# athas/raytracers

Measured on AMD Instinct MI355X. Metric: Mray/s (primary+secondary) on rgbbox & irreg 1000x1000, higher is better.
Workload: dtype f32

## Files before the change

### raytracers_amd/csrc/api.cpp

```cpp
#include <hip/hip_runtime.h>

#include <algorithm>
#include <chrono>
#include <cmath>
#include <cstdio>
#include <cstdlib>
#include <cstring>
#include <memory>
#include <string>
#include <vector>

#include "../../include/rt_mi355x.h"
#include "rt_device.hpp"
#include "rt_host.hpp"
#include "rt_internal.hpp"

namespace rti {
int fail(rt_context *ctx, const std::string &msg) {
  if (ctx) ctx->err = msg;
  return 1;
}
int hip_fail(rt_context *ctx, hipError_t e, const char *what) {
  return fail(ctx, std::string(what) + ": " + hipGetErrorString(e));
}
// ... 402 lines not shown
  p->dark = (ctx->dark_stop != 0 && p->cost == nullptr && (!instrumented || ctx->dark_stop > 0)) ? 1 : 0;
}

void set_leaf_box(const rt_context *ctx, const rt_prepared *ps, const Plan &pl, const float *cams_dev, bool instrumented, rtk::KParams *p) {
  p->leaf_box = 0;
  if (ctx->leaf_box == 0 || !ps->leaf.ok || pl.variant != RT_VARIANT_POOLED || (instrumented && ctx->leaf_box <= 0)) return;
  if (pl.lds_nodes != p->n_nodes || pl.lds_sph != p->n_sph) return;
  if (cams_dev == nullptr ? !rt::leaf_box_camera_ok(ps->leaf, &p->cam.ox) : (cams_dev != ctx->cams_dev || ctx->cams_host == nullptr)) return;
  for (int f = 0; cams_dev != nullptr && f < p->nframes; ++f)
    if (!rt::leaf_box_camera_ok(ps->leaf, ctx->cams_host + 12 * f)) return;
  rtk::PooledKey k{};
  if (!rtk::choose_pooled(*p, instrumented, pl.waves, 0, &k) || !rtk::pooled_leaf_box(k)) return;
  p->leaf_box = 1;
}

std::string pooled_launch_name(const rtk::KParams &p, int waves, int rays = 0) {
  rtk::PooledKey k{};
  return rtk::choose_pooled(p, false, waves, rays, &k) ? rtk::pooled_name(k) : "none";
}
const char *pooled_launch_nodes(const rtk::KParams &p, int waves) {
  rtk::PooledKey k{};
  return rtk::choose_pooled(p, false, waves, 0, &k) && rtk::pooled_presort(k) ? "sign-ordered" : "planes";
}

void frame_params(const rt_prepared *ps, int64_t h, int64_t w, int rows_per_tile, int part, int nparts, int max_depth, const float *cam12, rtk::KParams *p) {
  scene_params(ps, p);
  std::memcpy(&p->cam, cam12 ? static_cast<const void *>(cam12) : static_cast<const void *>(&ps->cam), sizeof(p->cam));
  p->w = static_cast<int>(w); p->h = static_cast<int>(h);
  p->rows_local = static_cast<int>(rt::part_rows(h, rows_per_tile, part, nparts));
  p->rows_per_tile = rows_per_tile; p->part = part; p->nparts = nparts;
  p->rpt_log2 = (rows_per_tile & (rows_per_tile - 1)) == 0 ? __builtin_ctz(rows_per_tile) : -1;
  p->tiles_x = (p->w + 7) / 8;
  p->tiles_y = (p->rows_local + 7) / 8;
  p->max_depth = max_depth;
  p->nframes = 1;
}

bool twenty_waves(const rt_context *ctx, const Plan &pl) { return pl.waves * (pl.grid_full / std::max(1, ctx->num_cu)) == 20; }

int pooled_shape_params(rt_context *ctx, const rt_prepared *ps, const Plan &pl, rtk::KParams *p) {
  p->static_first = ctx->static_first;
  p->lds_nodes = pl.lds_nodes; p->lds_sph = pl.lds_sph;
  p->smax = pl.smax; p->lmax = pl.lmax;
  p->thr_shade = ctx->thr_shade; p->thr_leaf = ctx->thr_leaf;
  p->capb = pl.capb; p->capl = pl.capl; p->ray_planes = pl.ray_planes;
  if (pl.spill_stride > 0) {
    if (int rc = ensure_spill(ctx, pl.spill_stride)) return rc;
    p->spill = ctx->spill_dev;
    p->spill_stride = pl.spill_stride;
  }
  p->prio_depth = ctx->prio_depth;
  p->box2 = ctx->box2;
  p->look_max = ctx->look_max > 0 ? ctx->look_max : (twenty_waves(ctx, pl) ? 16 : (p->nframes > 1 || p->nchunks > 16384) ? 32 : 64);
  p->tl_log2 = ps->tl_depth;
  return 0;
}

// ... 218 lines not shown
int rti::pooled_rays_params(rt_context *ctx, const rt_prepared *ps, const Plan &pl, rtk::KParams *pp) {
  rtk::KParams &p = *pp;
  if (ps->n >= (int64_t(1) << 22)) return fail(ctx, "pooled kernel: at most 2^22 spheres (work items and hit keys carry the leaf index in 22 bits)");
  const int64_t nblocks = (static_cast<int64_t>(p.nrays) + 63) / 64;
  p.nframes = 1;
  p.queue = ctx->queue_dev;
  p.w = 64; p.h = 1;
  p.rows_local = 1; p.rows_per_tile = 1; p.part = 0; p.nparts = 1; p.rpt_log2 = 0;
  p.tiles_x = static_cast<int>(nblocks); p.tiles_y = 1;
  p.nchunks = static_cast<int>(nblocks);
  p.tpt_log2 = 0;
  set_counters(&p, ctx->xcd_queues != 0 ? 2 : 0, pl.grid);
  return pooled_shape_params(ctx, ps, pl, &p);
}

int rti::launch_pooled_rays(rt_context *ctx, const rtk::KParams &p, const Plan &pl, int rays) {
  RT_HIP(ctx, rtk::launch_pooled(p, false, pl.grid, pl.waves, ctx->stream, rays));
  char buf[256];
  std::snprintf(buf, sizeof buf, "family=pooled tickets=rays instantiation=%s frames=1 tiles=%d grid=%d waves=%d counters=%d%s deep_class=0 deep_split=0 recording=0%s",
                pooled_launch_name(p, pl.waves, rays).c_str(), p.nchunks, pl.grid, pl.waves, p.nshards, p.interleave ? "(turns)" : "",
                p.ray_tlo_dev != nullptr ? " intervals=per-ray" : "");
  ctx->last_launch = buf;
  return 0;
}

int rti::enqueue_render(rt_context *ctx, const rt_prepared *ps, int64_t h, int64_t w, int32_t max_depth, int32_t rows_per_tile,
                        int32_t part, int32_t nparts, int32_t *out_dev, bool stats, const float *cam12, int32_t nframes,
                        int64_t frame_stride, const float *cams_dev, bool inplace) {
  if (!ctx || !ps) return fail(ctx, "null context or prepared scene");
  RT_LOCK(ctx);
  RT_LOCK_PS(ps);
// ... 72 lines not shown
    ctx->last_launch = "family=persistent";
    return 0;
  }
  if (ps->n >= (int64_t(1) << 22)) return fail(ctx, "pooled kernel: at most 2^22 spheres (work items and hit keys carry the leaf index in 22 bits)");
  if (p.rpt_log2 < 0) return fail(ctx, "pooled kernel: rows_per_tile must be a power of two");
  if (int rc = get_uv(ctx, w, h, &p.u_tab, &p.v_tab)) return rc;
  tick("uv tables");
  TileOrder *to = nullptr;
  if (ctx->adaptive_order && !p.cams)
    if (int rc = find_view(ctx, ps, p, pl, &to)) return rc;
  Tickets t;
  if (int rc = choose_tickets(ctx, ps, to, xq, tick, p, pl, &t)) return rc;
  set_cull(ctx, ps, pl, cams_dev, &p);
  set_dark(ctx, false, &p);
  set_leaf_box(ctx, ps, pl, cams_dev, false, &p);
  tick("before launch");
  RT_HIP(ctx, rtk::launch_pooled(p, false, pl.grid, pl.waves, ctx->stream));
  tick("launch_pooled");
  char buf[320];
  std::snprintf(buf, sizeof buf, "family=pooled tickets=%s%s instantiation=%s frames=%d tiles=%d grid=%d waves=%d counters=%d%s deep_class=%d deep_split=%d recording=%d nodes=%s,dark=%d,leaf_box=%d",
                p.px_hdr ? "pixel-list" : t.first_order ? "tiles-bit-reversed" : (p.order ? "tiles-ordered" : "tiles-raster"), t.borrowed ? "(borrowed)" : "",
                pooled_launch_name(p, pl.waves).c_str(), p.nframes, p.nchunks, pl.grid, pl.waves, p.nshards, p.interleave ? "(turns)" : "", p.px_hdr ? 0 : p.deep_class,
                p.px_hdr ? 0 : p.deep_split, p.cost ? (p.cost_px ? 2 : 1) : 0, pooled_launch_nodes(p, pl.waves), p.dark, p.leaf_box);
  ctx->last_launch = buf;
  if (to && p.cost) {
    to->sort_pending = true;
    to->sort_px = p.cost_px != nullptr;
    to->rec_out_skip = p.out_skip;
    if (ctx->eager_sort && (stream_was_idle || ctx->sync_policy))
      if (int rc = sort_view(ctx, ps, to, p, pl)) return rc;
    tick("record: eager sorts");
  }
  return 0;
}
using rti::enqueue_render;

extern "C" void rt_context_destroy(rt_context *ctx);

// ... 221 lines not shown
    ctx->px_solo_div = std::max(1, std::min(4096, v));
  } else if (k == "eager_sort") {
    drain_streams(ctx);
    ctx->eager_sort = v != 0;
  } else if (k == "borrow") {
    ctx->borrow = std::max(0, std::min(4, v));
  } else if (k == "stack_cap") {
    if (v != 0 && v != rtk::kSpillCapbTest) return fail(ctx, "stack_cap must be 0 or 192");
    ctx->stack_cap = v;
  } else if (k == "wide_waves") {
    ctx->wide_waves = std::max(0, std::min(2, v));
  } else if (k == "cull") {
    ctx->cull = std::max(-1, std::min(1, v));
  } else if (k == "dark_stop") {
    ctx->dark_stop = std::max(-1, std::min(1, v));
  } else if (k == "leaf_box") {
    ctx->leaf_box = std::max(-1, std::min(1, v));
  } else if (k == "sync_policy") {
    ctx->sync_policy = v != 0;
  } else {
    return fail(ctx, "unknown option: " + k);
  }
  return 0;
}

extern "C" int rt_context_device_info(const rt_context *ctx, int *device, int *num_cu, int *lds_bytes, char *name,
                                      int name_len) {
  RT_LOCK(const_cast<rt_context *>(ctx));
  if (!ctx) return 1;
  if (device) *device = ctx->device;
// ... 608 lines not shown
        p.deep_split = dp.deep_split;
        p.deep_cap_log2 = dp.cap_log2;
        if (dp.sparse && ctx->grid_div == 0) pl.grid = pl.grid_full;
        if (px_list_launch(ctx, p, pl, &o)) {
          p.px_list = o.px_list;
          p.px_hdr = reinterpret_cast<const int *>(o.px_list + o.px_elems);
          p.px_hold = ctx->px_hold;
          p.px_prio = ctx->px_prio;
          p.solo = (ctx->trace_solo && o.px_solo && ctx->solo && ps->tl_depth == rtk::kTreeletDepth) ? 1 : 0;
          if (ctx->grid_div == 0 && pl.grid != pl.grid_full && counters_follow(&p, xq, pl.grid_full)) pl.grid = pl.grid_full;
        }
      }
    nw = pl.grid * pl.waves;
    set_cull(ctx, ps, pl, nullptr, &p);
    set_dark(ctx, true, &p);
    set_leaf_box(ctx, ps, pl, nullptr, true, &p);
    e = rtk::launch_pooled(p, true, pl.grid, pl.waves, ctx->stream);
    if (e == hipSuccess) e = hipStreamSynchronize(ctx->stream);
    if (e == hipSuccess) e = hipMemcpy(records, trace, sizeof(unsigned long long) * rtk::kTraceWords * static_cast<size_t>(nw), hipMemcpyDeviceToHost);
  }
  (void)hipFree(tmp);
  (void)hipFree(trace);
  if (rc) return rc;
  if (e != hipSuccess) return hip_fail(ctx, e, "rt_render_trace");
  *num_waves = nw;
  return 0;
}

extern "C" int rt_render_timed(rt_context *ctx, const rt_prepared *ps, int64_t h, int64_t w, int32_t max_depth,
                               int32_t rows_per_tile, int32_t part, int32_t nparts, int32_t *out_dev, int32_t warmup,
// ... 58 lines not shown
```

### raytracers_amd/csrc/render_kernels.hip

```cpp
#include <hip/hip_runtime.h>

#include <mutex>
#include <type_traits>
#include <utility>

#include "lane_core.h"
#include "rt_device.hpp"
#include "treelet.h"

#ifdef RT_ISA_MARKS
#define RT_MARK(name) asm volatile("; RT_MARK " name)
#else
#define RT_MARK(name)
#endif

namespace rtk {

__device__ __forceinline__ int global_row(const KParams &p, int lrow) {
  const int k = lrow / p.rows_per_tile;
  return (k * p.nparts + p.part) * p.rows_per_tile + (lrow - k * p.rows_per_tile);
}

__device__ __forceinline__ size_t out_index(const KParams &p, int lrow, int col) {
  return (size_t)lrow * p.w + col + (size_t)(lrow / p.rows_per_tile) * (size_t)p.out_skip;
// ... 269 lines not shown
}

__device__ __forceinline__ float pull(int lane_byte, float v) {
  return __int_as_float(__builtin_amdgcn_ds_bpermute(lane_byte, __float_as_int(v)));
}

typedef const __attribute__((address_space(4))) KParams *KParamsArg;
typedef float v4f __attribute__((ext_vector_type(4)));
__device__ __forceinline__ float4 lds_load16(unsigned a) {
  const v4f v = *reinterpret_cast<const __attribute__((address_space(3))) v4f *>(a);
  return make_float4(v.x, v.y, v.z, v.w);
}
typedef float v2f __attribute__((ext_vector_type(2)));
typedef const __attribute__((address_space(3))) char *lds_cp;
__device__ __forceinline__ lds_cp lds_ptr(unsigned a) { return reinterpret_cast<lds_cp>(a); }
__device__ __forceinline__ v2f lds_load8(lds_cp a) { return *reinterpret_cast<const __attribute__((address_space(3))) v2f *>(a); }
__device__ __forceinline__ float lds_load4f(lds_cp a) { return *reinterpret_cast<const __attribute__((address_space(3))) float *>(a); }
#define RT_PS_NEAR(cell, t, entry) ((cell) + (t) + (entry))
#define RT_PS_FAR(cell, t, entry, dist) ((cell) - (t) + ((entry) + (int)(dist)))
__device__ __forceinline__ unsigned lds_load4(unsigned a) { return *reinterpret_cast<const __attribute__((address_space(3))) unsigned *>(a); }

constexpr bool kSoloCull = false;
template <bool CULL, bool TRACE = false>
__device__ __attribute__((noinline)) void solo_trace(KParamsArg pp_v, unsigned smem_lds, unsigned wbase_lds, float ox, float oy, float oz,
                                                     float dx, float dy, float dz, float lr, float lg, float lb, int pix, int depth,
                                                     int ptile) {
  const unsigned long long pp_bits = (unsigned long long)pp_v;
  KParamsArg pp = (KParamsArg)(((unsigned long long)(unsigned)uni((int)(pp_bits >> 32)) << 32) | (unsigned)uni((int)pp_bits));
  smem_lds = (unsigned)uni((int)smem_lds); wbase_lds = (unsigned)uni((int)wbase_lds);
  pix = uni(pix); depth = uni(depth); ptile = uni(ptile);
// ... 143 lines not shown
      return;
    }
  }
}

__device__ __forceinline__ int launch_dark() {
  return *reinterpret_cast<const volatile __attribute__((address_space(4))) int *>(&((KParamsArg)__builtin_amdgcn_kernarg_segment_ptr())->dark);
}

__device__ __forceinline__ unsigned long long launch_leaf_off() {
  KParamsArg kp = (KParamsArg)__builtin_amdgcn_kernarg_segment_ptr();
  asm volatile("" : "+s"(kp));
  return (unsigned long long)(unsigned)kp->leaf_box - 1ull;
}

template <int THREADS, bool ALL_LDS, bool STATS, bool SOLO, int TAIL = 0, bool ORD = false, bool CULL = false, int SPILL = 0, int RAYS = 0>
__global__ __launch_bounds__(THREADS, THREADS == 256 ? 5 : (THREADS / 64 + 3) / 4) void pooled_kernel(KParams p) {
  constexpr bool COLD = TAIL == 1, DONATE = TAIL == 2;
  constexpr bool ANY = RAYS == kRaysAny;
  static_assert(!RAYS || (!STATS && !SOLO && TAIL == 0 && !ORD && !CULL), "RAYS: the plain instantiations only");
  static_assert(!ORD || TAIL != 1, "ORD: no COLD variant");
  static_assert(!CULL || !ALL_LDS, "CULL: instantiated for the general scene path only");
  constexpr bool PRESORT = pooled_presort(ALL_LDS, SOLO, TAIL, ORD, RAYS);
  constexpr bool LEAFBOX = pooled_leaf_box(THREADS, ALL_LDS, STATS, SOLO, CULL, RAYS);
  extern __shared__ float4 smem[];
  const int lane = threadIdx.x & 63;
  const int wave = threadIdx.x >> 6;
  const int plane = p.lds_nodes;
  const int sph_base = 4 * plane;
  const int per_wave_dw = pooled_wave_dw(p.ray_planes, p.capb, p.capl);
  unsigned *const wbase = reinterpret_cast<unsigned *>(smem + sph_base + p.lds_sph) + wave * per_wave_dw;
  unsigned long long *const wkey = reinterpret_cast<unsigned long long *>(wbase);
  int *const wcnt = reinterpret_cast<int *>(wbase + 128);
  unsigned *const wdump = wbase + 192;
  float4 *const wray = reinterpret_cast<float4 *>(wbase + kPooledWaveFixedDw);
  unsigned *const wbox = wbase + kPooledWaveFixedDw + 256 * p.ray_planes;
  unsigned *const wleaf = wbox + p.capb;
  const __amdgpu_buffer_rsrc_t rs_nodes = make_rsrc(p.nodes64, (unsigned)p.n_nodes * 64u);
  const __amdgpu_buffer_rsrc_t rs_sph = make_rsrc(p.sph, (unsigned)p.n_sph * 16u);
  const __amdgpu_buffer_rsrc_t rs_col = make_rsrc(p.col, (unsigned)p.n_sph * 16u);

  if constexpr (PRESORT) {
    auto ref_of = [](float w) { const int c = f2i(w) >> 8; return (unsigned)(c < 0 ? c : c * kPsNodeBytes) << kPsItemShift; };
    for (int i = threadIdx.x; i < plane; i += THREADS) {
      const float4 ll = p.nodes64[4 * i], lh = p.nodes64[4 * i + 1], rl = p.nodes64[4 * i + 2], rh = p.nodes64[4 * i + 3];
      presort_pack(reinterpret_cast<unsigned *>(smem) + (kPsNodeBytes / 4) * i, &ll.x, &lh.x, &rl.x, &rh.x, ref_of(ll.w), ref_of(lh.w));
    }
  } else {
    for (int i = threadIdx.x; i < 4 * plane; i += THREADS) smem[(i & 3) * plane + (i >> 2)] = p.nodes64[i];
  }
  for (int i = threadIdx.x; i < p.lds_sph; i += THREADS) smem[sph_base + i] = p.sph[i];
  for (int i = lane; i < per_wave_dw; i += 64) wbase[i] = 0u;
  unsigned *const wg_words = reinterpret_cast<unsigned *>(smem + sph_base + p.lds_sph) + 193;
  if (DONATE && threadIdx.x == 0) wg_words[1] = THREADS / 64;
  __syncthreads();
  wkey[lane] = kKeyInit;

  Ray r = {};
  float lr = 1.0f, lg = 1.0f, lb = 1.0f;
  int depth = 0;
  int pix = -1;
  unsigned long long n_rays = 0, n_box = 0, n_sph = 0;
  int nbox = 0, nleaf = 0;
  static_assert(!SPILL || (THREADS == 256 && !ALL_LDS && !SOLO && TAIL == 0 && !ORD), "SPILL: the plain and CULL kernels of the four-wave workgroups");
  unsigned *const wspill = wbase + 193;
  auto spill_region = [&]() { return p.spill + (size_t)(blockIdx.x * (THREADS / 64) + wave) * (size_t)p.spill_stride; };
  unsigned q_next = 0, q_end = 0;
  int q_tile = 0;
// ... 140 lines not shown
          bool root = false;
          if (STATS) tr_ops[2]++;
          const unsigned long long tr_s0 = STATS ? clock64() : 0ull;
          if constexpr (ANY) {
            if (done) {
              p.occluded[pix] = wkey[lane] == kKeyAnyHit ? 1 : 0;
              pix = -1;
            }
          } else if (done) {
            if (STATS) tr_maxdepth = depth > tr_maxdepth ? depth : tr_maxdepth;
            const unsigned long long key = wkey[lane];
            const float best = __uint_as_float((unsigned)(key >> 32));
            const bool hit = key != kKeyInit;
            const int bestj = (int)((unsigned)key >> 1);
            const int wj = hit ? bestj : 0;
            float4 c = buf_load16(rs_col, wj * 16), s;
            if (ALL_LDS) {
              s = smem[sph_base + wj];
            } else {
              s = smem[sph_base + (wj < p.lds_sph ? wj : 0)];
              if (wj >= p.lds_sph) s = buf_load16(rs_sph, wj * 16);
            }
            if (!hit) {
              s = make_float4(0.f, 0.f, 0.f, 1.f);
              c = make_float4(0.f, 0.f, 0.f, 0.f);
            }
            bool have = hit;
            float t = best;
            if (hit && !rehit_is_best(best, ((unsigned)key & 1u) != 0u)) have = rehit_full(r, best, s.x, s.y, s.z, s.w, &t);
            int32_t pixel;
            if constexpr (!SPILL) pixel = 0;
            bool more;
            if constexpr (RAYS)
// ... 91 lines not shown
                exhausted = true;
                if (STATS) tr_exh = wall_clock64();
                break;
              }
              q_next = sp.q_next;
              q_end = sp.q_end;
              q_enter = true;
            }
            if (__builtin_expect(q_enter || (q_next & 63u) == 0u, 0)) {
              q_enter = false;
              unsigned t = q_next >> 6;
              if (p.nframes > 1) {
                unsigned f;
                if (p.order != nullptr) {
                  const int *cb = p.order + p.nchunks;
                  unsigned c = 0;
                  while (c + 1 < (unsigned)kOrderClasses && t >= (unsigned)p.nframes * (unsigned)cb[c + 1]) ++c;
                  const unsigned base = (unsigned)cb[c], size = (unsigned)cb[c + 1] - base;
                  const unsigned within = t - (unsigned)p.nframes * base;
                  f = within / size;
                  t = base + (within - f * size);
                } else {
                  f = t / (unsigned)p.nchunks;
                  t -= f * (unsigned)p.nchunks;
                }
                q_frame_off = (int)(f * (unsigned)p.frame_stride);
                if (p.cams != nullptr) q_cam = p.cams[f];
              }
              bool deep_tile;
              if (p.nshards == 1 || p.interleave) {
                q_tile = p.order != nullptr ? p.order[t] : (int)t;
                deep_tile = deep_on && (int)t < p.order[p.nchunks + p.deep_class];
              } else {
// ... 95 lines not shown
              }
            }
          }
          if (root) ray_derive(r);
          const bool root_hit = root && (ANY ? interval_ok(a_lo, a_hi) && box_hit_interval(r, p.root_lo[0], p.root_lo[1], p.root_lo[2], p.root_hi[0], p.root_hi[1], p.root_hi[2], a_lo, a_hi)
                                             : box_hit(r, p.root_lo[0], p.root_lo[1], p.root_lo[2], p.root_hi[0], p.root_hi[1], p.root_hi[2]));
          if (root) {
            wkey[lane] = ANY ? any_key_seed(a_hi) : kKeyInit;
            wcnt[lane] = root_hit ? 1 : 0;
            wray[lane] = make_float4(r.ox, r.oy, r.oz, r.a);
            wray[64 + lane] = make_float4(r.ix, r.iy, r.iz, CULL ? cull_weight(r, p.cull_c2) : ANY ? a_lo : 0.0f);
            if (p.ray_planes == 3) wray[128 + lane] = make_float4(r.dx, r.dy, r.dz, 0.0f);
            if (STATS) { n_rays++; n_box++; }
          }
          const unsigned long long m_root = bal(root_hit);
          if (root_hit) wbox[nbox + lane_rank(m_root)] = (unsigned)lane << 2 | (PRESORT ? sign_offsets(r) << 5 : 0u);
          nbox = uni(nbox + __popcll(m_root));
          if (p.prio_depth > 0 && !hold) {
            const bool live = pix >= 0;
            if (bal(live && depth >= 4 * p.prio_depth) != 0ull) __builtin_amdgcn_s_setprio(3);
            else if (bal(live && depth >= 2 * p.prio_depth) != 0ull) __builtin_amdgcn_s_setprio(2);
            else if (bal(live && depth >= p.prio_depth) != 0ull) __builtin_amdgcn_s_setprio(1);
            else __builtin_amdgcn_s_setprio(0);
          }
          if (STATS) tr_cyc[4] += clock64() - tr_s0;
          RT_MARK("SHADE_END");
          continue;
        }
      }
     }
     leaf_op = drain | (nbox == 0);
// ... 47 lines not shown
        if (STATS) { tr_ops[0]++; tr_items[0] += FULL ? 64 : nbox; }
        const int top = nbox - 1 - lane;
        const unsigned item = wbox[FULL ? top : (top < 0 ? 0 : top)];
        const unsigned long long m_act = FULL ? ~0ull : bal(top >= 0);
        nbox = uni(FULL ? nbox - 64 : 0);
        const int sl4 = (int)(item & 0xfcu);
        const int ni16 = (int)((item >> 4) & 0xfffffff0u);
        const float4 *const rayp = reinterpret_cast<const float4 *>(reinterpret_cast<const char *>(wray) + 4 * sl4);
        const float4 ra = rayp[0], ri = rayp[64];
        Ray q;
        q.ox = ra.x; q.oy = ra.y; q.oz = ra.z;
        q.ix = ri.x; q.iy = ri.y; q.iz = ri.z;
        int cl8, cr8;
        unsigned long long m_hl, m_hr;
        if constexpr (PRESORT) {
          const lds_cp cell = lds_ptr((unsigned)(size_t)smem + (item >> kPsItemShift));
          const int sn = (int)(item >> 5), tx = sn & (int)kSignX, ty = sn & (int)kSignY, tz = sn & (int)kSignZ;
          const v2f nx = lds_load8(RT_PS_NEAR(cell, tx, kPsX)), fx = lds_load8(RT_PS_FAR(cell, tx, kPsX, kSignX));
          const v2f ny = lds_load8(RT_PS_NEAR(cell, ty, kPsY)), fy = lds_load8(RT_PS_FAR(cell, ty, kPsY, kSignY));
          const v2f nz = lds_load8(RT_PS_NEAR(cell, tz, kPsZ)), fz = lds_load8(RT_PS_FAR(cell, tz, kPsZ, kSignZ));
          const v2f refs = lds_load8(cell + kPsRefs);
          asm volatile("" ::"v"(ra.w), "v"(ri.w));
          cl8 = f2i(refs.x); cr8 = f2i(refs.y);
          m_hl = bal(box_hit_presorted(q, nx.x, fx.x, ny.x, fy.x, nz.x, fz.x, 0.0f, kTMax));
          m_hr = bal(box_hit_presorted(q, nx.y, fx.y, ny.y, fy.y, nz.y, fz.y, 0.0f, kTMax));
        } else {
        float4 q0, q1, q2, q3;
        {
          const int lo16 = ALL_LDS ? ni16 : (ni16 < 16 * plane ? ni16 : 0);
          const float4 *const np = reinterpret_cast<const float4 *>(reinterpret_cast<const char *>(smem) + lo16);
          q0 = np[0]; q1 = np[plane]; q2 = np[2 * plane]; q3 = np[3 * plane];
// ... 43 lines not shown
        const unsigned item = wbox[top < 0 ? 0 : top];
        const bool act = top >= 0;
        nbox = uni(0);
        const int sl4 = (int)(item & 0xfcu);
        const int ni16 = (int)((item >> 4) & 0xfffffff0u);
        const float4 *const rayp = reinterpret_cast<const float4 *>(reinterpret_cast<const char *>(wray) + 4 * sl4);
        const float4 ra = rayp[0], ri = rayp[64];
        Ray q;
        q.ox = ra.x; q.oy = ra.y; q.oz = ra.z;
        q.ix = ri.x; q.iy = ri.y; q.iz = ri.z;
        int ref, cl8, cr8;
        bool pass, child_leaf, own;
        unsigned long long m_pass, m_cleaf, m_hl, m_hr;
        if constexpr (PRESORT) {
          const int sn = (int)(item >> 5), tx = sn & (int)kSignX, ty = sn & (int)kSignY, tz = sn & (int)kSignZ;
          const lds_cp cell = lds_ptr((unsigned)(size_t)smem + (item >> kPsItemShift) + 4u * (unsigned)role);
          const float cnx = lds_load4f(RT_PS_NEAR(cell, tx, kPsX)), cfx = lds_load4f(RT_PS_FAR(cell, tx, kPsX, kSignX));
          const float cny = lds_load4f(RT_PS_NEAR(cell, ty, kPsY)), cfy = lds_load4f(RT_PS_FAR(cell, ty, kPsY, kSignY));
          const float cnz = lds_load4f(RT_PS_NEAR(cell, tz, kPsZ)), cfz = lds_load4f(RT_PS_FAR(cell, tz, kPsZ, kSignZ));
          ref = f2i(lds_load4f(cell + kPsRefs));
          child_leaf = act & (ref < 0);
          own = box_hit_presorted(q, cnx, cfx, cny, cfy, cnz, cfz, 0.0f, kTMax);
          pass = act & (ref >= 0) & own;
          const lds_cp cell2 = lds_ptr((unsigned)(size_t)smem + (pass ? (unsigned)ref >> kPsItemShift : 0u));
          const v2f nx = lds_load8(RT_PS_NEAR(cell2, tx, kPsX)), fx = lds_load8(RT_PS_FAR(cell2, tx, kPsX, kSignX));
          const v2f ny = lds_load8(RT_PS_NEAR(cell2, ty, kPsY)), fy = lds_load8(RT_PS_FAR(cell2, ty, kPsY, kSignY));
          const v2f nz = lds_load8(RT_PS_NEAR(cell2, tz, kPsZ)), fz = lds_load8(RT_PS_FAR(cell2, tz, kPsZ, kSignZ));
          const v2f refs = lds_load8(cell2 + kPsRefs);
          asm volatile("" ::"v"(ra.w), "v"(ri.w));
          cl8 = f2i(refs.x); cr8 = f2i(refs.y);
          m_pass = bal(pass); m_cleaf = bal(child_leaf);
          m_hl = bal(box_hit_presorted(q, nx.x, fx.x, ny.x, fy.x, nz.x, fz.x, 0.0f, kTMax));
          m_hr = bal(box_hit_presorted(q, nx.y, fx.y, ny.y, fy.y, nz.y, fz.y, 0.0f, kTMax));
        } else {
        float4 lo, hi;
        {
          const bool res = ALL_LDS || ni16 < 16 * plane;
          const int lo16 = res ? ni16 : 0;
          const char *const np = reinterpret_cast<const char *>(smem) + lo16;
// ... 477 lines not shown
  return hipGetLastError();
}

hipError_t launch_persistent(const KParams &p, bool stats, int grid, int waves_per_wg, hipStream_t stream) {
  if (grid <= 0) return hipSuccess;
  if (stats) return launch_persistent_t<512, true>(p, grid, stream);
  switch (waves_per_wg) {
  case 4: return launch_persistent_t<256, false>(p, grid, stream);
  case 8: return launch_persistent_t<512, false>(p, grid, stream);
  case 12: return launch_persistent_t<768, false>(p, grid, stream);
  case 16: return launch_persistent_t<1024, false>(p, grid, stream);
  default: return hipErrorInvalidValue;
  }
}

size_t pooled_lds_bytes(int lds_nodes, int lds_sph, int capb, int capl, int ray_planes, int waves_per_wg) {
  return (size_t)lds_nodes * 64 + (size_t)lds_sph * 16 + (size_t)waves_per_wg * pooled_wave_dw(ray_planes, capb, capl) * sizeof(unsigned);
}

template <int I>
static auto pooled_fn() {
  constexpr const PooledKey &k = kPooledKeys[I];
  return pooled_kernel<k.threads, k.all_lds, k.stats, k.solo, k.tail, k.ord, k.cull, k.spill, k.rays>;
}

template <int I>
static hipError_t launch_pooled_t(const KParams &p, int grid, hipStream_t stream) {
  constexpr int threads = kPooledKeys[I].threads;
  const size_t lds = pooled_lds_bytes(p.lds_nodes, p.lds_sph, p.capb, p.capl, p.ray_planes, threads / 64);
  auto kfn = pooled_fn<I>();
  if (hipError_t e = allow_full_lds(reinterpret_cast<const void *>(kfn)); e != hipSuccess) return e;
  hipLaunchKernelGGL(kfn, dim3(grid), dim3(threads), lds, stream, p);
  return hipGetLastError();
}

template <int... I>
static hipError_t launch_pooled_key(const PooledKey &k, const KParams &p, int grid, hipStream_t stream, std::integer_sequence<int, I...>) {
  hipError_t e = hipErrorInvalidValue;
  (void)((kPooledKeys[I] == k && ((e = launch_pooled_t<I>(p, grid, stream)), true)) || ...);
  return e;
}

hipError_t launch_pooled(const KParams &p, bool stats, int grid, int waves_per_wg, hipStream_t stream, int rays) {
  if (rays == kRaysAny && p.occluded == nullptr) return hipErrorInvalidValue;
// ... 66 lines not shown
```

### raytracers_amd/csrc/rt_device.hpp

```cpp
#pragma once
#include <hip/hip_runtime.h>
#include <stdint.h>

#include <string>

#include "lane_core.h"
#include "treelet.h"

namespace rtk {

constexpr int kTraceWords = 16;
constexpr int kStackPixel = 64;
constexpr int kPooledWaveFixedDw = 128 + 64 + 4;
constexpr int pooled_wave_dw(int ray_planes, int capb, int capl) { return kPooledWaveFixedDw + 256 * ray_planes + capb + capl; }
constexpr int kSpillCapb = 1088, kSpillCapbTest = 192;

constexpr int kQueueStride = 32;
constexpr int kMaxShards = 8;
constexpr int kQueueExit = kQueueStride * kMaxShards;
constexpr int kQueueDwords = kQueueStride * (kMaxShards + 1);
constexpr int kOrderTableDw = 16;
constexpr int order_table_ints(int ntiles) { return ntiles + kOrderTableDw * kMaxShards; }

struct Shard {
  int x0, sw;
  int seg;
  int ntiles;
};
__host__ __device__ inline Shard shard_of(int s, int ns_log2, int tiles_x, int tiles_y) {
// ... 173 lines not shown
  const unsigned *px_list;
  int px_hold;
  int px_prio;
  int cull;
  float cull_c2;
  float cull_kappa;
  int dark;
  const float *u_tab;
  const float *v_tab;
  unsigned *spill;
  int spill_stride;
  int leaf_box;
  const float *rays;
  float *colour3;
  int nrays;
  unsigned char *occluded;
  float ray_tlo, ray_thi;
  const float *ray_tlo_dev, *ray_thi_dev;
};

#if defined(__HIPCC__)
__device__ __forceinline__ int f2i(float f) { return __float_as_int(f); }

typedef int v4i __attribute__((ext_vector_type(4)));
__device__ __forceinline__ __amdgpu_buffer_rsrc_t make_rsrc(const void *base, unsigned bytes) {
  return __builtin_amdgcn_make_buffer_rsrc(const_cast<void *>(base), 0, (int)bytes, 0x00020000);
}
__device__ __forceinline__ float4 buf_load16(__amdgpu_buffer_rsrc_t rsrc, int byte_off) {
  const v4i v = __builtin_amdgcn_raw_buffer_load_b128(rsrc, byte_off, 0, 0);
  return make_float4(__int_as_float(v.x), __int_as_float(v.y), __int_as_float(v.z), __int_as_float(v.w));
// ... 71 lines not shown
    if (waves_per_wg != 16 || p.nframes != 1) return false;
    k.ord = true; k.solo = p.solo != 0; k.tail = p.donate ? 2 : 0;
    k.all_lds = all_lds && !k.cull;
  } else {
    k.solo = p.solo && p.nframes == 1 && p.order != nullptr && p.deep_class > 0 && p.deep_split == 6 && p.tl_log2 == kTreeletDepth;
    if (waves_per_wg == 16) k.tail = p.cold ? 1 : p.donate ? 2 : 0;
    else if (waves_per_wg != 4 && waves_per_wg != 8 && waves_per_wg != 12) return false;
    k.all_lds = all_lds && !k.cull;
  }
  *out = k;
  return true;
}

constexpr bool pooled_presort(bool all_lds, bool solo, int tail, bool ord, int rays) { return all_lds && !solo && tail == 0 && !ord && rays == 0; }
constexpr bool pooled_presort(const PooledKey &k) { return pooled_presort(k.all_lds, k.solo, k.tail, k.ord, k.rays); }

constexpr bool pooled_leaf_box(int threads, bool all_lds, bool stats, bool solo, bool cull, int rays) {
  return rays == 0 && !cull && (stats || (all_lds && !(threads == 256 && solo)));
}
constexpr bool pooled_leaf_box(const PooledKey &k) { return pooled_leaf_box(k.threads, k.all_lds, k.stats, k.solo, k.cull, k.rays); }

inline std::string pooled_name(const PooledKey &k) {
  std::string s = k.rays == kRaysAny ? "any" : k.ord ? "ORD" : k.tail == 1 ? "COLD" : k.tail == 2 ? "DONATE" : "";
  if (k.solo) s += s.empty() ? "SOLO" : "+SOLO";
  if (k.ord && k.tail == 2) s += "+DONATE";
  if (s.empty()) s = "plain";
  if (k.cull) s += "+CULL";
  if (k.spill) s += "+SPILL";
  return s;
}

hipError_t launch_pixel(const KParams &p, bool stats, hipStream_t stream);
hipError_t launch_pixel_rays(const KParams &p, hipStream_t stream);
hipError_t launch_persistent(const KParams &p, bool stats, int grid, int waves_per_wg, hipStream_t stream);
size_t persistent_lds_bytes(int lds_nodes, int lds_sph, int smax, int lmax, int waves_per_wg);
hipError_t launch_pooled(const KParams &p, bool stats, int grid, int waves_per_wg, hipStream_t stream, int rays = 0);
size_t pooled_lds_bytes(int lds_nodes, int lds_sph, int capb, int capl, int ray_planes, int waves_per_wg);
struct GpuBvhOut {
  float *L7;
  float *bmin, *bmax;
  int *left, *right, *parent;
  float4 *nodes32;
  float4 *nodes64;
  float4 *sph, *col;
  int *ids;
};
void warm_render_kernels();
hipError_t warm_scratch(hipStream_t stream, int *sink_dev);
void warm_build_kernels();
size_t gpu_build_scratch_bytes(int n);
hipError_t gpu_copy_from_pinned(void *dst_dev, const void *src_pinned, size_t bytes, hipStream_t stream);
size_t gpu_build_pinned_bytes();
// ... 43 lines not shown
```

### raytracers_amd/csrc/rt_internal.hpp

```cpp
#pragma once
#include <hip/hip_runtime.h>

#include <cstdint>
#include <future>
#include <mutex>
#include <string>
#include <vector>

#include "../../include/rt_mi355x.h"
#include "rt_device.hpp"
#include "rt_host.hpp"

struct rt_group;

struct rt_context {
  std::recursive_mutex mu;
  int device = 0;
  hipStream_t stream = nullptr;
  bool own_stream = false;
  std::string err;
  bool synced_since_render = true;
  std::string last_launch;
  int num_cu = 0;
  int lds_bytes = 0;
  std::string name;
  int variant = RT_VARIANT_AUTO;
  int waves_per_wg = 0;
  int wgs_per_cu = 1;
  int thr_shade = 40;
  int thr_leaf = 24;
  int lmax = 8;
  int lds_scene_bytes = -1;
  int lds_sph_first = 0;
  int handover = 1;
  int donate_max = 64;
  int look_max = 0;
  int box2 = 1;
  int solo = 1;
  int treelet = rtk::kTreeletDepth;
  int trace_solo = 0;
  int trace_part = 0, trace_nparts = 1;
  int ray_planes = 0;
  int gpu_build = 1;
  int prio_depth = 4;
  int grid_div = 0;
  int adaptive_order = 1;
  int deep_class = -1;
// ... 191 lines not shown
```

Baseline: 21490.

## Stage sphere colours in LDS and unroll order-class lookup in pooled kernel

Adds an optional path that copies the per-sphere colour array into LDS next to the sphere data when the whole scene fits, so shading reads colours from LDS instead of global buffer loads. Presorted node references now carry absolute LDS offsets, which drops an add per node fetch. The tile-order class search becomes an unrolled register scan for the simpler kernel variants. The cost is more LDS per workgroup, which could limit residency, plus extra copy work at kernel start.

Measured after the change: 21700, median of 6. About the same (+1.0%).

```diff
diff --git a/raytracers_amd/csrc/api.cpp b/raytracers_amd/csrc/api.cpp
--- a/raytracers_amd/csrc/api.cpp
+++ b/raytracers_amd/csrc/api.cpp
@@ -440,6 +440,18 @@
   p->leaf_box = 1;
 }
 
+void set_lds_col(const rt_context *ctx, const Plan &pl, bool instrumented, int rays, rtk::KParams *p) {
+  p->lds_col = 0;
+  rtk::PooledKey k{};
+  if (ctx->lds_col == 0 || pl.variant != RT_VARIANT_POOLED || !rtk::choose_pooled(*p, instrumented, pl.waves, rays, &k) || !rtk::pooled_lds_col(k)) return;
+  const int wgs = std::max(1, pl.grid_full / std::max(1, ctx->num_cu));
+  const int64_t scene = int64_t(16) * rtk::pooled_scene_f4(rtk::pooled_presort(k), p->lds_nodes, p->lds_sph, p->n_sph);
+  const int64_t waves = int64_t(4) * pl.waves * rtk::pooled_wave_dw(p->ray_planes, p->capb, p->capl);
+  if (scene + waves > std::min(ctx->lds_bytes, 160 * 1024) / wgs - 512) return;
+  if (ctx->lds_scene_bytes >= 0 && scene > ctx->lds_scene_bytes) return;
+  p->lds_col = p->n_sph;
+}
+
 std::string pooled_launch_name(const rtk::KParams &p, int waves, int rays = 0) {
   rtk::PooledKey k{};
   return rtk::choose_pooled(p, false, waves, rays, &k) ? rtk::pooled_name(k) : "none";
@@ -467,6 +479,7 @@
 int pooled_shape_params(rt_context *ctx, const rt_prepared *ps, const Plan &pl, rtk::KParams *p) {
   p->static_first = ctx->static_first;
   p->lds_nodes = pl.lds_nodes; p->lds_sph = pl.lds_sph;
+  p->lds_col = 0;
   p->smax = pl.smax; p->lmax = pl.lmax;
   p->thr_shade = ctx->thr_shade; p->thr_leaf = ctx->thr_leaf;
   p->capb = pl.capb; p->capl = pl.capl; p->ray_planes = pl.ray_planes;
@@ -715,7 +728,9 @@
   return pooled_shape_params(ctx, ps, pl, &p);
 }
 
-int rti::launch_pooled_rays(rt_context *ctx, const rtk::KParams &p, const Plan &pl, int rays) {
+int rti::launch_pooled_rays(rt_context *ctx, const rtk::KParams &p_in, const Plan &pl, int rays) {
+  rtk::KParams p = p_in;
+  set_lds_col(ctx, pl, false, rays, &p);
   RT_HIP(ctx, rtk::launch_pooled(p, false, pl.grid, pl.waves, ctx->stream, rays));
   char buf[256];
   std::snprintf(buf, sizeof buf, "family=pooled tickets=rays instantiation=%s frames=1 tiles=%d grid=%d waves=%d counters=%d%s deep_class=0 deep_split=0 recording=0%s",
@@ -818,14 +833,15 @@
   set_cull(ctx, ps, pl, cams_dev, &p);
   set_dark(ctx, false, &p);
   set_leaf_box(ctx, ps, pl, cams_dev, false, &p);
+  set_lds_col(ctx, pl, false, 0, &p);
   tick("before launch");
   RT_HIP(ctx, rtk::launch_pooled(p, false, pl.grid, pl.waves, ctx->stream));
   tick("launch_pooled");
-  char buf[320];
-  std::snprintf(buf, sizeof buf, "family=pooled tickets=%s%s instantiation=%s frames=%d tiles=%d grid=%d waves=%d counters=%d%s deep_class=%d deep_split=%d recording=%d nodes=%s,dark=%d,leaf_box=%d",
+  char buf[352];
+  std::snprintf(buf, sizeof buf, "family=pooled tickets=%s%s instantiation=%s frames=%d tiles=%d grid=%d waves=%d counters=%d%s deep_class=%d deep_split=%d recording=%d nodes=%s,dark=%d,lds_col=%d,leaf_box=%d",
                 p.px_hdr ? "pixel-list" : t.first_order ? "tiles-bit-reversed" : (p.order ? "tiles-ordered" : "tiles-raster"), t.borrowed ? "(borrowed)" : "",
                 pooled_launch_name(p, pl.waves).c_str(), p.nframes, p.nchunks, pl.grid, pl.waves, p.nshards, p.interleave ? "(turns)" : "", p.px_hdr ? 0 : p.deep_class,
-                p.px_hdr ? 0 : p.deep_split, p.cost ? (p.cost_px ? 2 : 1) : 0, pooled_launch_nodes(p, pl.waves), p.dark, p.leaf_box);
+                p.px_hdr ? 0 : p.deep_split, p.cost ? (p.cost_px ? 2 : 1) : 0, pooled_launch_nodes(p, pl.waves), p.dark, p.lds_col != 0, p.leaf_box);
   ctx->last_launch = buf;
   if (to && p.cost) {
     to->sort_pending = true;
@@ -1077,6 +1093,8 @@
     ctx->cull = std::max(-1, std::min(1, v));
   } else if (k == "dark_stop") {
     ctx->dark_stop = std::max(-1, std::min(1, v));
+  } else if (k == "lds_col") {
+    ctx->lds_col = v != 0;
   } else if (k == "leaf_box") {
     ctx->leaf_box = std::max(-1, std::min(1, v));
   } else if (k == "sync_policy") {
@@ -1715,6 +1733,7 @@
     nw = pl.grid * pl.waves;
     set_cull(ctx, ps, pl, nullptr, &p);
     set_dark(ctx, true, &p);
+    set_lds_col(ctx, pl, true, 0, &p);
     set_leaf_box(ctx, ps, pl, nullptr, true, &p);
     e = rtk::launch_pooled(p, true, pl.grid, pl.waves, ctx->stream);
     if (e == hipSuccess) e = hipStreamSynchronize(ctx->stream);
diff --git a/raytracers_amd/csrc/render_kernels.hip b/raytracers_amd/csrc/render_kernels.hip
--- a/raytracers_amd/csrc/render_kernels.hip
+++ b/raytracers_amd/csrc/render_kernels.hip
@@ -307,6 +307,7 @@
 typedef float v2f __attribute__((ext_vector_type(2)));
 typedef const __attribute__((address_space(3))) char *lds_cp;
 __device__ __forceinline__ lds_cp lds_ptr(unsigned a) { return reinterpret_cast<lds_cp>(a); }
+__device__ __forceinline__ unsigned lds_offset(const void *q) { return (unsigned)(size_t)(lds_cp)q; }
 __device__ __forceinline__ v2f lds_load8(lds_cp a) { return *reinterpret_cast<const __attribute__((address_space(3))) v2f *>(a); }
 __device__ __forceinline__ float lds_load4f(lds_cp a) { return *reinterpret_cast<const __attribute__((address_space(3))) float *>(a); }
 #define RT_PS_NEAR(cell, t, entry) ((cell) + (t) + (entry))
@@ -480,6 +481,12 @@
   return (unsigned long long)(unsigned)kp->leaf_box - 1ull;
 }
 
+__device__ __forceinline__ int launch_lds_col() {
+  KParamsArg kp = (KParamsArg)__builtin_amdgcn_kernarg_segment_ptr();
+  asm volatile("" : "+s"(kp));
+  return kp->lds_col;
+}
+
 template <int THREADS, bool ALL_LDS, bool STATS, bool SOLO, int TAIL = 0, bool ORD = false, bool CULL = false, int SPILL = 0, int RAYS = 0>
 __global__ __launch_bounds__(THREADS, THREADS == 256 ? 5 : (THREADS / 64 + 3) / 4) void pooled_kernel(KParams p) {
   constexpr bool COLD = TAIL == 1, DONATE = TAIL == 2;
@@ -493,9 +500,11 @@
   const int lane = threadIdx.x & 63;
   const int wave = threadIdx.x >> 6;
   const int plane = p.lds_nodes;
-  const int sph_base = 4 * plane;
+  const int sph_base = pooled_scene_f4(PRESORT, plane, 0, 0);
+  constexpr bool LDSCOL = pooled_lds_col(ALL_LDS, SOLO, TAIL, ORD, RAYS);
+  const int col_f4 = LDSCOL ? p.lds_col : 0;
   const int per_wave_dw = pooled_wave_dw(p.ray_planes, p.capb, p.capl);
-  unsigned *const wbase = reinterpret_cast<unsigned *>(smem + sph_base + p.lds_sph) + wave * per_wave_dw;
+  unsigned *const wbase = reinterpret_cast<unsigned *>(smem + sph_base + p.lds_sph + col_f4) + wave * per_wave_dw;
   unsigned long long *const wkey = reinterpret_cast<unsigned long long *>(wbase);
   int *const wcnt = reinterpret_cast<int *>(wbase + 128);
   unsigned *const wdump = wbase + 192;
@@ -507,7 +516,8 @@
   const __amdgpu_buffer_rsrc_t rs_col = make_rsrc(p.col, (unsigned)p.n_sph * 16u);
 
   if constexpr (PRESORT) {
-    auto ref_of = [](float w) { const int c = f2i(w) >> 8; return (unsigned)(c < 0 ? c : c * kPsNodeBytes) << kPsItemShift; };
+    const int ps_base = (int)lds_offset(smem);
+    auto ref_of = [ps_base](float w) { const int c = f2i(w) >> 8; return (unsigned)(c < 0 ? c : c * kPsNodeBytes + ps_base) << kPsItemShift; };
     for (int i = threadIdx.x; i < plane; i += THREADS) {
       const float4 ll = p.nodes64[4 * i], lh = p.nodes64[4 * i + 1], rl = p.nodes64[4 * i + 2], rh = p.nodes64[4 * i + 3];
       presort_pack(reinterpret_cast<unsigned *>(smem) + (kPsNodeBytes / 4) * i, &ll.x, &lh.x, &rl.x, &rh.x, ref_of(ll.w), ref_of(lh.w));
@@ -516,8 +526,10 @@
     for (int i = threadIdx.x; i < 4 * plane; i += THREADS) smem[(i & 3) * plane + (i >> 2)] = p.nodes64[i];
   }
   for (int i = threadIdx.x; i < p.lds_sph; i += THREADS) smem[sph_base + i] = p.sph[i];
+  if constexpr (LDSCOL)
+    for (int i = threadIdx.x; i < col_f4; i += THREADS) smem[sph_base + p.lds_sph + i] = p.col[i];
   for (int i = lane; i < per_wave_dw; i += 64) wbase[i] = 0u;
-  unsigned *const wg_words = reinterpret_cast<unsigned *>(smem + sph_base + p.lds_sph) + 193;
+  unsigned *const wg_words = reinterpret_cast<unsigned *>(smem + sph_base + p.lds_sph + col_f4) + 193;
   if (DONATE && threadIdx.x == 0) wg_words[1] = THREADS / 64;
   __syncthreads();
   wkey[lane] = kKeyInit;
@@ -688,9 +700,15 @@
             const bool hit = key != kKeyInit;
             const int bestj = (int)((unsigned)key >> 1);
             const int wj = hit ? bestj : 0;
-            float4 c = buf_load16(rs_col, wj * 16), s;
+            float4 c, s;
+            if constexpr (!LDSCOL) c = buf_load16(rs_col, wj * 16);
             if (ALL_LDS) {
               s = smem[sph_base + wj];
+              if constexpr (LDSCOL) {
+                const int lc = launch_lds_col();
+                if (lc != 0) c = smem[sph_base + lc + wj];
+                else c = buf_load16(rs_col, wj * 16);
+              }
             } else {
               s = smem[sph_base + (wj < p.lds_sph ? wj : 0)];
               if (wj >= p.lds_sph) s = buf_load16(rs_sph, wj * 16);
@@ -812,9 +830,21 @@
                 unsigned f;
                 if (p.order != nullptr) {
                   const int *cb = p.order + p.nchunks;
-                  unsigned c = 0;
-                  while (c + 1 < (unsigned)kOrderClasses && t >= (unsigned)p.nframes * (unsigned)cb[c + 1]) ++c;
-                  const unsigned base = (unsigned)cb[c], size = (unsigned)cb[c + 1] - base;
+                  unsigned base, next;
+                  if constexpr (SPILL != 0 || SOLO || TAIL != 0) {
+                    unsigned c = 0;
+                    while (c + 1 < (unsigned)kOrderClasses && t >= (unsigned)p.nframes * (unsigned)cb[c + 1]) ++c;
+                    base = (unsigned)cb[c]; next = (unsigned)cb[c + 1];
+                  } else {
+                    int cbv[kOrderClasses + 1];
+#pragma unroll
+                    for (int k = 0; k <= kOrderClasses; ++k) cbv[k] = cb[k];
+                    base = (unsigned)cbv[0]; next = (unsigned)cbv[1];
+#pragma unroll
+                    for (int k = 1; k < kOrderClasses; ++k)
+                      if (t >= (unsigned)p.nframes * (unsigned)cbv[k]) { base = (unsigned)cbv[k]; next = (unsigned)cbv[k + 1]; }
+                  }
+                  const unsigned size = next - base;
                   const unsigned within = t - (unsigned)p.nframes * base;
                   f = within / size;
                   t = base + (within - f * size);
@@ -940,7 +970,7 @@
             if (STATS) { n_rays++; n_box++; }
           }
           const unsigned long long m_root = bal(root_hit);
-          if (root_hit) wbox[nbox + lane_rank(m_root)] = (unsigned)lane << 2 | (PRESORT ? sign_offsets(r) << 5 : 0u);
+          if (root_hit) wbox[nbox + lane_rank(m_root)] = (unsigned)lane << 2 | (PRESORT ? sign_offsets(r) << 5 | lds_offset(smem) << kPsItemShift : 0u);
           nbox = uni(nbox + __popcll(m_root));
           if (p.prio_depth > 0 && !hold) {
             const bool live = pix >= 0;
@@ -1018,7 +1048,7 @@
         int cl8, cr8;
         unsigned long long m_hl, m_hr;
         if constexpr (PRESORT) {
-          const lds_cp cell = lds_ptr((unsigned)(size_t)smem + (item >> kPsItemShift));
+          const lds_cp cell = lds_ptr(item >> kPsItemShift);
           const int sn = (int)(item >> 5), tx = sn & (int)kSignX, ty = sn & (int)kSignY, tz = sn & (int)kSignZ;
           const v2f nx = lds_load8(RT_PS_NEAR(cell, tx, kPsX)), fx = lds_load8(RT_PS_FAR(cell, tx, kPsX, kSignX));
           const v2f ny = lds_load8(RT_PS_NEAR(cell, ty, kPsY)), fy = lds_load8(RT_PS_FAR(cell, ty, kPsY, kSignY));
@@ -1092,7 +1122,7 @@
         unsigned long long m_pass, m_cleaf, m_hl, m_hr;
         if constexpr (PRESORT) {
           const int sn = (int)(item >> 5), tx = sn & (int)kSignX, ty = sn & (int)kSignY, tz = sn & (int)kSignZ;
-          const lds_cp cell = lds_ptr((unsigned)(size_t)smem + (item >> kPsItemShift) + 4u * (unsigned)role);
+          const lds_cp cell = lds_ptr((item >> kPsItemShift) + 4u * (unsigned)role);
           const float cnx = lds_load4f(RT_PS_NEAR(cell, tx, kPsX)), cfx = lds_load4f(RT_PS_FAR(cell, tx, kPsX, kSignX));
           const float cny = lds_load4f(RT_PS_NEAR(cell, ty, kPsY)), cfy = lds_load4f(RT_PS_FAR(cell, ty, kPsY, kSignY));
           const float cnz = lds_load4f(RT_PS_NEAR(cell, tz, kPsZ)), cfz = lds_load4f(RT_PS_FAR(cell, tz, kPsZ, kSignZ));
@@ -1100,7 +1130,7 @@
           child_leaf = act & (ref < 0);
           own = box_hit_presorted(q, cnx, cfx, cny, cfy, cnz, cfz, 0.0f, kTMax);
           pass = act & (ref >= 0) & own;
-          const lds_cp cell2 = lds_ptr((unsigned)(size_t)smem + (pass ? (unsigned)ref >> kPsItemShift : 0u));
+          const lds_cp cell2 = lds_ptr(pass ? (unsigned)ref >> kPsItemShift : lds_offset(smem));
           const v2f nx = lds_load8(RT_PS_NEAR(cell2, tx, kPsX)), fx = lds_load8(RT_PS_FAR(cell2, tx, kPsX, kSignX));
           const v2f ny = lds_load8(RT_PS_NEAR(cell2, ty, kPsY)), fy = lds_load8(RT_PS_FAR(cell2, ty, kPsY, kSignY));
           const v2f nz = lds_load8(RT_PS_NEAR(cell2, tz, kPsZ)), fz = lds_load8(RT_PS_FAR(cell2, tz, kPsZ, kSignZ));
@@ -1608,8 +1638,8 @@
   }
 }
 
-size_t pooled_lds_bytes(int lds_nodes, int lds_sph, int capb, int capl, int ray_planes, int waves_per_wg) {
-  return (size_t)lds_nodes * 64 + (size_t)lds_sph * 16 + (size_t)waves_per_wg * pooled_wave_dw(ray_planes, capb, capl) * sizeof(unsigned);
+size_t pooled_lds_bytes(int lds_nodes, int lds_sph, int capb, int capl, int ray_planes, int waves_per_wg, bool presort, int lds_col) {
+  return (size_t)pooled_scene_f4(presort, lds_nodes, lds_sph, lds_col) * 16 + (size_t)waves_per_wg * pooled_wave_dw(ray_planes, capb, capl) * sizeof(unsigned);
 }
 
 template <int I>
@@ -1621,7 +1651,9 @@
 template <int I>
 static hipError_t launch_pooled_t(const KParams &p, int grid, hipStream_t stream) {
   constexpr int threads = kPooledKeys[I].threads;
-  const size_t lds = pooled_lds_bytes(p.lds_nodes, p.lds_sph, p.capb, p.capl, p.ray_planes, threads / 64);
+  if (p.lds_col != 0 && (!pooled_lds_col(kPooledKeys[I]) || p.lds_col != p.n_sph)) return hipErrorInvalidValue;
+  const size_t lds = pooled_lds_bytes(p.lds_nodes, p.lds_sph, p.capb, p.capl, p.ray_planes, threads / 64, pooled_presort(kPooledKeys[I]), p.lds_col);
+  if (lds > 160 * 1024) return hipErrorInvalidValue;
   auto kfn = pooled_fn<I>();
   if (hipError_t e = allow_full_lds(reinterpret_cast<const void *>(kfn)); e != hipSuccess) return e;
   hipLaunchKernelGGL(kfn, dim3(grid), dim3(threads), lds, stream, p);
diff --git a/raytracers_amd/csrc/rt_device.hpp b/raytracers_amd/csrc/rt_device.hpp
--- a/raytracers_amd/csrc/rt_device.hpp
+++ b/raytracers_amd/csrc/rt_device.hpp
@@ -13,6 +13,9 @@
 constexpr int kStackPixel = 64;
 constexpr int kPooledWaveFixedDw = 128 + 64 + 4;
 constexpr int pooled_wave_dw(int ray_planes, int capb, int capl) { return kPooledWaveFixedDw + 256 * ray_planes + capb + capl; }
+constexpr int pooled_scene_f4(bool presort, int lds_nodes, int lds_sph, int lds_col) {
+  return (presort ? (kPsNodeBytes * lds_nodes + 15) / 16 : 4 * lds_nodes) + lds_sph + lds_col;
+}
 constexpr int kSpillCapb = 1088, kSpillCapbTest = 192;
 
 constexpr int kQueueStride = 32;
@@ -216,6 +219,7 @@
   const float *rays;
   float *colour3;
   int nrays;
+  int lds_col;
   unsigned char *occluded;
   float ray_tlo, ray_thi;
   const float *ray_tlo_dev, *ray_thi_dev;
@@ -317,6 +321,8 @@
 
 constexpr bool pooled_presort(bool all_lds, bool solo, int tail, bool ord, int rays) { return all_lds && !solo && tail == 0 && !ord && rays == 0; }
 constexpr bool pooled_presort(const PooledKey &k) { return pooled_presort(k.all_lds, k.solo, k.tail, k.ord, k.rays); }
+constexpr bool pooled_lds_col(bool all_lds, bool solo, int tail, bool ord, int rays) { return pooled_presort(all_lds, solo, tail, ord, rays); }
+constexpr bool pooled_lds_col(const PooledKey &k) { return pooled_lds_col(k.all_lds, k.solo, k.tail, k.ord, k.rays); }
 
 constexpr bool pooled_leaf_box(int threads, bool all_lds, bool stats, bool solo, bool cull, int rays) {
   return rays == 0 && !cull && (stats || (all_lds && !(threads == 256 && solo)));
@@ -338,7 +344,7 @@
 hipError_t launch_persistent(const KParams &p, bool stats, int grid, int waves_per_wg, hipStream_t stream);
 size_t persistent_lds_bytes(int lds_nodes, int lds_sph, int smax, int lmax, int waves_per_wg);
 hipError_t launch_pooled(const KParams &p, bool stats, int grid, int waves_per_wg, hipStream_t stream, int rays = 0);
-size_t pooled_lds_bytes(int lds_nodes, int lds_sph, int capb, int capl, int ray_planes, int waves_per_wg);
+size_t pooled_lds_bytes(int lds_nodes, int lds_sph, int capb, int capl, int ray_planes, int waves_per_wg, bool presort = false, int lds_col = 0);
 struct GpuBvhOut {
   float *L7;
   float *bmin, *bmax;
diff --git a/raytracers_amd/csrc/rt_internal.hpp b/raytracers_amd/csrc/rt_internal.hpp
--- a/raytracers_amd/csrc/rt_internal.hpp
+++ b/raytracers_amd/csrc/rt_internal.hpp
@@ -31,6 +31,7 @@
   int thr_leaf = 24;
   int lmax = 8;
   int lds_scene_bytes = -1;
+  int lds_col = 1;
   int lds_sph_first = 0;
   int handover = 1;
   int donate_max = 64;
```
